# sun-huangqingbo/multiplexed-image-annotator

Hardware: AMD Instinct MI355X
Metric: cells/sec annotated (whole node) (higher is better)
Workload: dtype f16

## Files before the change

multiplexed-image-annotator_amd/csrc/cell_attention.hip:

```cpp

#include "gemm_epi.h"
#include "ribca_common.h"
#include "ribca_kernels.h"

namespace ribca {

namespace {

typedef __attribute__((__vector_size__(4 * sizeof(_Float16)))) _Float16 f16x4c;
typedef __attribute__((__vector_size__(4 * sizeof(short)))) short s16x4c;
__device__ __forceinline__ f16x4c lds_read_tr16c(const char* p) {
  return __builtin_bit_cast(f16x4c, __builtin_amdgcn_ds_read_tr16_b64_v4i16((s16x4c __attribute__((address_space(3)))*)(p)));
}

constexpr int kTP = 112, kVRows = 128;

template <int D, int HD> struct CellGeom {
  static constexpr int Dp = (D + 31) / 32 * 32;
  static constexpr int NK = Dp / 32;
  static constexpr int GD = HD == 32 ? 64 : 48;
  static constexpr int NTP = GD / 16;
  static constexpr int WROWS = 3 * GD;
  static constexpr int WSTAGE = WROWS * ROWB;
  static constexpr int GROUPS = D / GD;
  static constexpr int HPG = GD / HD;
  static constexpr int KIMG = kTP * ROWB;
  static constexpr int VROWB = 4 * GD;
  static constexpr int VIMG = kVRows * VROWB + 64;
  static constexpr int CB = 2 * 3 * D * 4;
  static constexpr int RING = 3;
  static constexpr int OFF_K = RING * WSTAGE;
  static constexpr int OFF_V = OFF_K + HPG * KIMG;
  static constexpr int OFF_CB = OFF_V + (VIMG + 15) / 16 * 16;
  static constexpr int LDS = OFF_CB + CB;
  static_assert(D % GD == 0 && GD % HD == 0 && HD % 4 == 0 && HD <= 32 && HPG % 2 == 0 && WROWS % 8 == 0, "head geometry");
};

}

template <int D, int HD>
__global__ __launch_bounds__(512) void cell_qkv_attention_kernel(const uint16_t* __restrict__ z, int ldz, const uint16_t* __restrict__ W, int ldw,
                                                                 const float* __restrict__ bias2, const float* __restrict__ csum,
                                                                 const float2* __restrict__ rowstat, uint16_t* __restrict__ out, int ldo, int T,
                                                                 float scale) {
  using G = CellGeom<D, HD>;
  constexpr int NK = G::NK, GROUPS = G::GROUPS, HPG = G::HPG, kRing = G::RING, kGroupDims = G::GD, NTP = G::NTP, kWStage = G::WSTAGE;
  constexpr int NTILES = 3 * NTP;
  constexpr int TOTAL = GROUPS * NK;
  constexpr int GPL = G::WROWS / 8;
  extern __shared__ __attribute__((aligned(16))) char smem[];
  const int tid = threadIdx.x, lane = tid & 63;
  const int wave = __builtin_amdgcn_readfirstlane(tid >> 6);
  const int cell = blockIdx.x;
  const int r16 = lane & 15, g = lane >> 4;

  for (int i = tid; i < 3 * D / 4; i += 512) {
    reinterpret_cast<float4*>(smem + G::OFF_CB)[i] = reinterpret_cast<const float4*>(csum)[i];
    reinterpret_cast<float4*>(smem + G::OFF_CB + 3 * D * 4)[i] = reinterpret_cast<const float4*>(bias2)[i];
  }
  for (int o = kTP * G::VROWB + tid * 16; o < G::VIMG; o += 512 * 16) *reinterpret_cast<uint4*>(smem + G::OFF_V + o) = uint4{0u, 0u, 0u, 0u};
  __syncthreads();

  if (wave == 7) {
    auto issue = [&](int step) {
      const int hg = step / NK, s = step - hg * NK;
      char* st = smem + (step % kRing) * kWStage;
#pragma unroll
      for (int i = 0; i < GPL; ++i) {
        const int row = i * 8 + (lane >> 3);
        const int which = row / kGroupDims, c = row - which * kGroupDims;
        const int n = which * D + hg * kGroupDims + c;
        const int ch = (lane & 7) ^ swz_f(row);
        const uint16_t* src = W + (size_t)n * ldw + s * (2 * BK) + ch * 8;
        __builtin_amdgcn_global_load_lds((const __attribute__((address_space(1))) void*)src, (__attribute__((address_space(3))) void*)(st + i * 1024), 16,
                                         0, 0);
      }
    };
    issue(0);
    issue(1);
    for (int step = 0; step < TOTAL; ++step) {
      if (step + 1 < TOTAL) wait_vmcnt<GPL>();
      else wait_vmcnt<0>();
      __builtin_amdgcn_s_barrier();
      asm volatile("" ::: "memory");
      if (step + 2 < TOTAL) issue(step + 2);
      if ((step + 1) % NK == 0) __builtin_amdgcn_s_barrier();
    }
    return;
  }

  const int tok = wave * 16 + r16;
  const int trow = tok < T ? tok : T - 1;
  const uint16_t* zr = z + ((size_t)cell * T + trow) * ldz;
  f16x8 ahi[NK], alo[NK];
#pragma unroll
  for (int s = 0; s < NK; ++s) {
    const uint4* p = reinterpret_cast<const uint4*>(zr + (4 * s + g) * 16);
    ahi[s] = __builtin_bit_cast(f16x8, p[0]);
    alo[s] = __builtin_bit_cast(f16x8, p[1]);
  }
  const float2 rs = rowstat[(size_t)cell * T + trow];
  const float rstd = rs.x, nm = -rs.y * rs.x;
  const char* cb = smem + G::OFF_CB;
  uint16_t* orow = out + ((size_t)cell * T + tok) * ldo;
  int w_rd[NTILES];
#pragma unroll
  for (int j = 0; j < NTILES; ++j) w_rd[j] = lds_off(16 * j + r16, 2 * g);
  const int k_wr = lds_off(tok, 2 * g);
  constexpr int KST = 4, NT = 7;

  int step = 0;
  for (int hg = 0; hg < GROUPS; ++hg) {
    f32x4 acc[NTILES];
#pragma unroll
    for (int j = 0; j < NTILES; ++j) acc[j] = f32x4{0.f, 0.f, 0.f, 0.f};
#pragma unroll
    for (int s = 0; s < NK; ++s, ++step) {
      asm volatile("s_waitcnt lgkmcnt(0)" ::: "memory");
      __builtin_amdgcn_s_barrier();
      asm volatile("" ::: "memory");
      const char* st = smem + (step % kRing) * kWStage;
#pragma unroll
      for (int jb = 0; jb < NTILES / 3; ++jb) {
        f16x8 whi[3], wlo[3];
#pragma unroll
        for (int j = 0; j < 3; ++j) {
          whi[j] = __builtin_bit_cast(f16x8, *reinterpret_cast<const uint4*>(st + w_rd[3 * jb + j]));
          wlo[j] = __builtin_bit_cast(f16x8, *reinterpret_cast<const uint4*>(st + (w_rd[3 * jb + j] ^ 16)));
        }
#pragma unroll
        for (int j = 0; j < 3; ++j) acc[3 * jb + j] = mfma_f16(wlo[j], ahi[s], acc[3 * jb + j]);
#pragma unroll
        for (int j = 0; j < 3; ++j) acc[3 * jb + j] = mfma_f16(whi[j], alo[s], acc[3 * jb + j]);
#pragma unroll
        for (int j = 0; j < 3; ++j) acc[3 * jb + j] = mfma_f16(whi[j], ahi[s], acc[3 * jb + j]);
      }
    }
#pragma unroll
    for (int j = 0; j < NTILES; ++j) {
      const int n = (j / NTP) * D + hg * kGroupDims + 16 * (j % NTP) + 4 * g;
      const float4 c4 = *reinterpret_cast<const float4*>(cb + n * 4), b4 = *reinterpret_cast<const float4*>(cb + 3 * D * 4 + n * 4);
      const f32x2v r2 = {rstd, rstd}, n2 = {nm, nm};
      const f32x2v lo2 = fma2(r2, f32x2v{acc[j][0], acc[j][1]}, fma2(n2, f32x2v{c4.x, c4.y}, f32x2v{b4.x, b4.y}));
      const f32x2v hi2 = fma2(r2, f32x2v{acc[j][2], acc[j][3]}, fma2(n2, f32x2v{c4.z, c4.w}, f32x2v{b4.z, b4.w}));
      acc[j] = f32x4{lo2.x, lo2.y, hi2.x, hi2.y};
    }
    f16x8 qhi[HPG], qlo[HPG];
#pragma unroll
    for (int h = 0; h < HPG; ++h) {
      constexpr int dummy = 0; (void)dummy;
      const int d_lo = h * HD, d_hi = d_lo + HD;
      const int tA = d_lo / 16, tB = (d_hi - 1) / 16;
      const bool inA = 16 * tA + 4 * g >= d_lo && 16 * tA + 4 * g < d_hi;
      const bool inB = tB != tA && 16 * tB + 4 * g >= d_lo && 16 * tB + 4 * g < d_hi;
      float qa[4], qb[4], ka[4], kb[4];
#pragma unroll
      for (int r = 0; r < 4; ++r) {
        qa[r] = inA ? acc[tA][r] * scale : 0.f;
        qb[r] = inB ? acc[tB][r] * scale : 0.f;
        ka[r] = inA ? acc[NTP + tA][r] : 0.f;
        kb[r] = inB ? acc[NTP + tB][r] : 0.f;
      }
      uint2 h0, l0, h1, l1;
      split4(qa, h0, l0);
      split4(qb, h1, l1);
      qhi[h] = __builtin_bit_cast(f16x8, uint4{h0.x, h0.y, h1.x, h1.y});
      qlo[h] = __builtin_bit_cast(f16x8, uint4{l0.x, l0.y, l1.x, l1.y});
      split4(ka, h0, l0);
      split4(kb, h1, l1);
      char* kimg = smem + G::OFF_K + h * G::KIMG;
      *reinterpret_cast<uint4*>(kimg + k_wr) = uint4{h0.x, h0.y, h1.x, h1.y};
      *reinterpret_cast<uint4*>(kimg + (k_wr ^ 16)) = uint4{l0.x, l0.y, l1.x, l1.y};
    }
    {
      uint16_t* vrow = reinterpret_cast<uint16_t*>(smem + G::OFF_V + tok * G::VROWB);
#pragma unroll
      for (int j = 0; j < NTP; ++j) {
        const float v4[4] = {acc[2 * NTP + j][0], acc[2 * NTP + j][1], acc[2 * NTP + j][2], acc[2 * NTP + j][3]};
        const int jj = kGroupDims == 64 ? (j ^ (tok & 3)) : j;
        ps_store4_pair<16>(vrow, 16 * jj + 4 * g, v4);
      }
    }
    asm volatile("s_waitcnt lgkmcnt(0)" ::: "memory");
    __builtin_amdgcn_s_barrier();
    asm volatile("" ::: "memory");

    constexpr int DT = (HD + 15) / 16;
    const char* vimg = smem + G::OFF_V;
#pragma unroll
    for (int hp = 0; hp < HPG; hp += 2) {
      f32x4 s[2][2 * KST];
#pragma unroll
      for (int kt = 0; kt < NT; ++kt) {
        const int ko = lds_off(16 * kt + r16, 2 * g);
#pragma unroll
        for (int e = 0; e < 2; ++e) {
          const char* kimg = smem + G::OFF_K + (hp + e) * G::KIMG;
          const f16x8 kh = __builtin_bit_cast(f16x8, *reinterpret_cast<const uint4*>(kimg + ko));
          const f16x8 kl = __builtin_bit_cast(f16x8, *reinterpret_cast<const uint4*>(kimg + (ko ^ 16)));
          s[e][kt] = f32x4{0.f, 0.f, 0.f, 0.f};
          s[e][kt] = mfma_f16(kl, qhi[hp + e], s[e][kt]);
          s[e][kt] = mfma_f16(kh, qlo[hp + e], s[e][kt]);
          s[e][kt] = mfma_f16(kh, qhi[hp + e], s[e][kt]);
        }
      }
      f16x8 phi[2][KST], plo[2][KST];
#pragma unroll
      for (int e = 0; e < 2; ++e) {
#pragma unroll
        for (int r = 0; r < 4; ++r)
          if (16 * (NT - 1) + 4 * g + r >= T) s[e][NT - 1][r] = -INFINITY;
        float mx = -INFINITY;
#pragma unroll
        for (int kt = 0; kt < NT; ++kt)
#pragma unroll
          for (int r = 0; r < 4; ++r) mx = fmaxf(mx, s[e][kt][r]);
        mx = fmaxf(mx, __shfl_xor(mx, 16, 64));
        mx = fmaxf(mx, __shfl_xor(mx, 32, 64));
        const f32x2v l2 = {1.44269504089f, 1.44269504089f}, moff = {-mx * 1.44269504089f, -mx * 1.44269504089f};
        f32x2v sum2 = {0.f, 0.f};
#pragma unroll
        for (int kt = 0; kt < NT; ++kt) {
          const f32x2v a0 = fma2(f32x2v{s[e][kt][0], s[e][kt][1]}, l2, moff);
          const f32x2v a1 = fma2(f32x2v{s[e][kt][2], s[e][kt][3]}, l2, moff);
          const f32x2v e0 = {__builtin_amdgcn_exp2f(a0.x), __builtin_amdgcn_exp2f(a0.y)}, e1 = {__builtin_amdgcn_exp2f(a1.x), __builtin_amdgcn_exp2f(a1.y)};
          s[e][kt] = f32x4{e0.x, e0.y, e1.x, e1.y};
          sum2 += e0;
          sum2 += e1;
        }
        float sum = sum2.x + sum2.y;
        sum += __shfl_xor(sum, 16, 64);
        sum += __shfl_xor(sum, 32, 64);
        const float inv = 1.0f / sum;
        const f32x2v inv2 = {inv, inv};
        s[e][NT] = f32x4{0.f, 0.f, 0.f, 0.f};
#pragma unroll
        for (int t = 0; t < KST; ++t) {
          const f32x2v pa0 = f32x2v{s[e][2 * t][0], s[e][2 * t][1]} * inv2, pa1 = f32x2v{s[e][2 * t][2], s[e][2 * t][3]} * inv2;
          const f32x2v pb0 = f32x2v{s[e][2 * t + 1][0], s[e][2 * t + 1][1]} * inv2, pb1 = f32x2v{s[e][2 * t + 1][2], s[e][2 * t + 1][3]} * inv2;
          const float pa[4] = {pa0.x, pa0.y, pa1.x, pa1.y}, pb[4] = {pb0.x, pb0.y, pb1.x, pb1.y};
          uint2 ha, la, hb, lb;
          split4_unit(pa, ha, la);
          split4_unit(pb, hb, lb);
          phi[e][t] = __builtin_bit_cast(f16x8, uint4{ha.x, ha.y, hb.x, hb.y});
          plo[e][t] = __builtin_bit_cast(f16x8, uint4{la.x, la.y, lb.x, lb.y});
        }
      }
#pragma unroll
      for (int dt = 0; dt < DT; ++dt) {
        f32x4 o[2] = {f32x4{0.f, 0.f, 0.f, 0.f}, f32x4{0.f, 0.f, 0.f, 0.f}};
#pragma unroll
        for (int t = 0; t < KST; ++t) {
#pragma unroll
          for (int e = 0; e < 2; ++e) {
            const int dcol0 = (hp + e) * HD + 16 * dt + 4 * (r16 & 3);
            const int dcol = kGroupDims == 64 ? ((((dcol0 >> 4) ^ (r16 >> 2)) << 4) | (dcol0 & 15)) : dcol0;
            const int voff = (dcol >> 3) * 32 + (dcol & 7) * 2;
            const char* va = vimg + (32 * t + 4 * g + (r16 >> 2)) * G::VROWB + voff;
            const f16x4c h0 = lds_read_tr16c(va), l0 = lds_read_tr16c(va + 16);
            const f16x4c h1 = lds_read_tr16c(va + 16 * G::VROWB), l1 = lds_read_tr16c(va + 16 * G::VROWB + 16);
            const f16x8 vhi = __builtin_shufflevector(h0, h1, 0, 1, 2, 3, 4, 5, 6, 7);
            const f16x8 vlo = __builtin_shufflevector(l0, l1, 0, 1, 2, 3, 4, 5, 6, 7);
            o[e] = mfma_f16(vlo, phi[e][t], o[e]);
            o[e] = mfma_f16(vhi, plo[e][t], o[e]);
            o[e] = mfma_f16(vhi, phi[e][t], o[e]);
          }
        }
        const int d = 16 * dt + 4 * g;
        if (tok < T && d < HD) {
#pragma unroll
          for (int e = 0; e < 2; ++e) {
            const float v4[4] = {o[e][0], o[e][1], o[e][2], o[e][3]};
            ps_store4(orow, (hg * HPG + hp + e) * HD + d, v4);
          }
        }
      }
    }
  }
}

bool cell_attention_supported(int D, int H, int T) { return H == kHeads && T == kTokens && (D == 144 || D == 288 || D == 384); }

void launch_cell_qkv_attention(const uint16_t* z, int ldz, const uint16_t* W, int ldw, const float* bias2, const float* csum, const float2* rowstat,
                               uint16_t* out, int ldo, int cells, int D, float scale, hipStream_t s) {
  if (cells <= 0) return;
  auto go = [&](auto kern, int lds) {
    static unsigned long long attr_done[3] = {0ull, 0ull, 0ull};
    const int slot = D == 288 ? 1 : D == 384 ? 2 : 0;
    if (!ensure_dynamic_lds(reinterpret_cast<const void*>(kern), lds, attr_done[slot])) return;
    hipLaunchKernelGGL(kern, dim3(cells), dim3(512), lds, s, z, ldz, W, ldw, bias2, csum, rowstat, out, ldo, (int)kTokens, scale);
  };
  if (D == 288) go(cell_qkv_attention_kernel<288, 24>, CellGeom<288, 24>::LDS);
  else if (D == 384) go(cell_qkv_attention_kernel<384, 32>, CellGeom<384, 32>::LDS);
  else go(cell_qkv_attention_kernel<144, 12>, CellGeom<144, 12>::LDS);
}

}
```

Measured before the change: 17400.

## Make cell attention kernel persistent and deepen weight ring for HD=24

Launches one workgroup per CU, and each workgroup loops over cells with a grid stride. The loader wave streams weights continuously across cell boundaries, so the ring no longer refills from empty for every cell. For HD=24 the ring grows to 5 stages, with counted vmcnt waits that keep more loads in flight, and LDS address arithmetic is simplified. The costs are more LDS use, which static asserts check against 160 KB, and fewer resident blocks, which may hurt load balance at the tail.

```diff
diff --git a/multiplexed-image-annotator_amd/csrc/cell_attention.hip b/multiplexed-image-annotator_amd/csrc/cell_attention.hip
--- a/multiplexed-image-annotator_amd/csrc/cell_attention.hip
+++ b/multiplexed-image-annotator_amd/csrc/cell_attention.hip
@@ -1,3 +1,5 @@
+
+#include <type_traits>
 
 #include "gemm_epi.h"
 #include "ribca_common.h"
@@ -28,12 +30,14 @@
   static constexpr int VROWB = 4 * GD;
   static constexpr int VIMG = kVRows * VROWB + 64;
   static constexpr int CB = 2 * 3 * D * 4;
-  static constexpr int RING = 3;
+  static constexpr int RING = HD == 24 ? 5 : 3;
   static constexpr int OFF_K = RING * WSTAGE;
   static constexpr int OFF_V = OFF_K + HPG * KIMG;
   static constexpr int OFF_CB = OFF_V + (VIMG + 15) / 16 * 16;
   static constexpr int LDS = OFF_CB + CB;
   static_assert(D % GD == 0 && GD % HD == 0 && HD % 4 == 0 && HD <= 32 && HPG % 2 == 0 && WROWS % 8 == 0, "head geometry");
+  static_assert(LDS <= 160 * 1024, "one workgroup per CU: the ring, the K / V images and the fold vectors share 160 KB of LDS");
+  static_assert(RING >= 3 && (RING - 2) * (WROWS / 8) <= 63 && NK >= RING - 2, "the loader's counted wait: RING - 2 younger stages in a 6-bit vmcnt");
 };
 
 }
@@ -42,16 +46,16 @@
 __global__ __launch_bounds__(512) void cell_qkv_attention_kernel(const uint16_t* __restrict__ z, int ldz, const uint16_t* __restrict__ W, int ldw,
                                                                  const float* __restrict__ bias2, const float* __restrict__ csum,
                                                                  const float2* __restrict__ rowstat, uint16_t* __restrict__ out, int ldo, int T,
-                                                                 float scale) {
+                                                                 int cells, float scale) {
   using G = CellGeom<D, HD>;
   constexpr int NK = G::NK, GROUPS = G::GROUPS, HPG = G::HPG, kRing = G::RING, kGroupDims = G::GD, NTP = G::NTP, kWStage = G::WSTAGE;
   constexpr int NTILES = 3 * NTP;
-  constexpr int TOTAL = GROUPS * NK;
   constexpr int GPL = G::WROWS / 8;
+  constexpr int kTopUp = kRing - 3;
   extern __shared__ __attribute__((aligned(16))) char smem[];
   const int tid = threadIdx.x, lane = tid & 63;
   const int wave = __builtin_amdgcn_readfirstlane(tid >> 6);
-  const int cell = blockIdx.x;
+  const int cell0 = blockIdx.x, cstride = gridDim.x;
   const int r16 = lane & 15, g = lane >> 4;
 
   for (int i = tid; i < 3 * D / 4; i += 512) {
@@ -62,37 +66,62 @@
   __syncthreads();
 
   if (wave == 7) {
-    auto issue = [&](int step) {
-      const int hg = step / NK, s = step - hg * NK;
-      char* st = smem + (step % kRing) * kWStage;
+    const int total = ((cells - 1 - cell0) / cstride + 1) * (GROUPS * NK);
+    int issued = 0, i_slot = 0, i_hg = 0, i_s = 0;
+    auto issue = [&]() {
+      if (issued == total) return;
+      char* st = smem + i_slot * kWStage;
 #pragma unroll
       for (int i = 0; i < GPL; ++i) {
         const int row = i * 8 + (lane >> 3);
         const int which = row / kGroupDims, c = row - which * kGroupDims;
-        const int n = which * D + hg * kGroupDims + c;
+        const int n = which * D + i_hg * kGroupDims + c;
         const int ch = (lane & 7) ^ swz_f(row);
-        const uint16_t* src = W + (size_t)n * ldw + s * (2 * BK) + ch * 8;
+        const uint16_t* src = W + (size_t)n * ldw + i_s * (2 * BK) + ch * 8;
         __builtin_amdgcn_global_load_lds((const __attribute__((address_space(1))) void*)src, (__attribute__((address_space(3))) void*)(st + i * 1024), 16,
                                          0, 0);
       }
+      ++issued;
+      i_slot = i_slot + 1 == kRing ? 0 : i_slot + 1;
+      if (++i_s == NK) {
+        i_s = 0;
+        i_hg = i_hg + 1 == GROUPS ? 0 : i_hg + 1;
+      }
     };
-    issue(0);
-    issue(1);
-    for (int step = 0; step < TOTAL; ++step) {
-      if (step + 1 < TOTAL) wait_vmcnt<GPL>();
-      else wait_vmcnt<0>();
+#pragma unroll
+    for (int e = 0; e < kRing - 1; ++e) issue();
+    auto step_barrier = [&](auto younger, bool request) {
+      if (issued == total) wait_vmcnt<0>();
+      else wait_vmcnt<decltype(younger)::value * GPL>();
       __builtin_amdgcn_s_barrier();
       asm volatile("" ::: "memory");
-      if (step + 2 < TOTAL) issue(step + 2);
-      if ((step + 1) % NK == 0) __builtin_amdgcn_s_barrier();
+      if (request) issue();
+    };
+    static_assert(kTopUp >= 0 && kTopUp <= 2, "the lead-draining steps are written out below");
+    for (int left = total; left > 0; left -= NK) {
+      if constexpr (kTopUp >= 1) step_barrier(std::integral_constant<int, kRing - 2>{}, false);
+      if constexpr (kTopUp >= 2) step_barrier(std::integral_constant<int, kRing - 3>{}, false);
+#pragma unroll
+      for (int i = kTopUp; i < NK; ++i) step_barrier(std::integral_constant<int, 1>{}, true);
+      __builtin_amdgcn_s_barrier();
+      asm volatile("" ::: "memory");
+#pragma unroll
+      for (int e = 0; e < kTopUp; ++e) issue();
     }
     return;
   }
 
   const int tok = wave * 16 + r16;
   const int trow = tok < T ? tok : T - 1;
+  f16x8 ahi[NK], alo[NK];
+  const char* cb = smem + G::OFF_CB;
+  const int w_rd0 = lds_off(r16, 2 * g), w_rd1 = w_rd0 ^ 16;
+  const int k_wr = lds_off(tok, 2 * g);
+  constexpr int KST = 4, NT = 7;
+
+  int slot = 0;
+  for (int cell = cell0; cell < cells; cell += cstride) {
   const uint16_t* zr = z + ((size_t)cell * T + trow) * ldz;
-  f16x8 ahi[NK], alo[NK];
 #pragma unroll
   for (int s = 0; s < NK; ++s) {
     const uint4* p = reinterpret_cast<const uint4*>(zr + (4 * s + g) * 16);
@@ -100,33 +129,29 @@
     alo[s] = __builtin_bit_cast(f16x8, p[1]);
   }
   const float2 rs = rowstat[(size_t)cell * T + trow];
-  const float rstd = rs.x, nm = -rs.y * rs.x;
-  const char* cb = smem + G::OFF_CB;
+  float rstd = rs.x, nm = -rs.y * rs.x;
+#pragma unroll
+  for (int s = 0; s < NK; ++s) asm volatile("" : "+v"(ahi[s]), "+v"(alo[s]));
+  asm volatile("" : "+v"(rstd), "+v"(nm));
   uint16_t* orow = out + ((size_t)cell * T + tok) * ldo;
-  int w_rd[NTILES];
-#pragma unroll
-  for (int j = 0; j < NTILES; ++j) w_rd[j] = lds_off(16 * j + r16, 2 * g);
-  const int k_wr = lds_off(tok, 2 * g);
-  constexpr int KST = 4, NT = 7;
-
-  int step = 0;
   for (int hg = 0; hg < GROUPS; ++hg) {
     f32x4 acc[NTILES];
 #pragma unroll
     for (int j = 0; j < NTILES; ++j) acc[j] = f32x4{0.f, 0.f, 0.f, 0.f};
 #pragma unroll
-    for (int s = 0; s < NK; ++s, ++step) {
+    for (int s = 0; s < NK; ++s) {
       asm volatile("s_waitcnt lgkmcnt(0)" ::: "memory");
       __builtin_amdgcn_s_barrier();
       asm volatile("" ::: "memory");
-      const char* st = smem + (step % kRing) * kWStage;
+      const char* st = smem + slot * kWStage;
+      slot = slot + 1 == kRing ? 0 : slot + 1;
 #pragma unroll
       for (int jb = 0; jb < NTILES / 3; ++jb) {
         f16x8 whi[3], wlo[3];
 #pragma unroll
         for (int j = 0; j < 3; ++j) {
-          whi[j] = __builtin_bit_cast(f16x8, *reinterpret_cast<const uint4*>(st + w_rd[3 * jb + j]));
-          wlo[j] = __builtin_bit_cast(f16x8, *reinterpret_cast<const uint4*>(st + (w_rd[3 * jb + j] ^ 16)));
+          whi[j] = __builtin_bit_cast(f16x8, *reinterpret_cast<const uint4*>(st + w_rd0 + (3 * jb + j) * 16 * ROWB));
+          wlo[j] = __builtin_bit_cast(f16x8, *reinterpret_cast<const uint4*>(st + w_rd1 + (3 * jb + j) * 16 * ROWB));
         }
 #pragma unroll
         for (int j = 0; j < 3; ++j) acc[3 * jb + j] = mfma_f16(wlo[j], ahi[s], acc[3 * jb + j]);
@@ -192,12 +217,11 @@
       f32x4 s[2][2 * KST];
 #pragma unroll
       for (int kt = 0; kt < NT; ++kt) {
-        const int ko = lds_off(16 * kt + r16, 2 * g);
 #pragma unroll
         for (int e = 0; e < 2; ++e) {
           const char* kimg = smem + G::OFF_K + (hp + e) * G::KIMG;
-          const f16x8 kh = __builtin_bit_cast(f16x8, *reinterpret_cast<const uint4*>(kimg + ko));
-          const f16x8 kl = __builtin_bit_cast(f16x8, *reinterpret_cast<const uint4*>(kimg + (ko ^ 16)));
+          const f16x8 kh = __builtin_bit_cast(f16x8, *reinterpret_cast<const uint4*>(kimg + w_rd0 + kt * 16 * ROWB));
+          const f16x8 kl = __builtin_bit_cast(f16x8, *reinterpret_cast<const uint4*>(kimg + w_rd1 + kt * 16 * ROWB));
           s[e][kt] = f32x4{0.f, 0.f, 0.f, 0.f};
           s[e][kt] = mfma_f16(kl, qhi[hp + e], s[e][kt]);
           s[e][kt] = mfma_f16(kh, qlo[hp + e], s[e][kt]);
@@ -277,9 +301,25 @@
       }
     }
   }
+  }
 }
 
 bool cell_attention_supported(int D, int H, int T) { return H == kHeads && T == kTokens && (D == 144 || D == 288 || D == 384); }
+
+static int device_cu_count() {
+  static int cached[64] = {};
+  int dev = 0;
+  if (hipGetDevice(&dev) != hipSuccess) dev = 0;
+  if (dev >= 0 && dev < 64 && cached[dev] > 0) return cached[dev];
+  int n = 0;
+  const hipError_t e = hipDeviceGetAttribute(&n, hipDeviceAttributeMultiprocessorCount, dev);
+  if (e != hipSuccess || n <= 0) {
+    launch_error("hipDeviceGetAttribute(MultiprocessorCount) failed on device %d: %s", dev, hipGetErrorString(e));
+    return 0;
+  }
+  if (dev >= 0 && dev < 64) cached[dev] = n;
+  return n;
+}
 
 void launch_cell_qkv_attention(const uint16_t* z, int ldz, const uint16_t* W, int ldw, const float* bias2, const float* csum, const float2* rowstat,
                                uint16_t* out, int ldo, int cells, int D, float scale, hipStream_t s) {
@@ -288,7 +328,9 @@
     static unsigned long long attr_done[3] = {0ull, 0ull, 0ull};
     const int slot = D == 288 ? 1 : D == 384 ? 2 : 0;
     if (!ensure_dynamic_lds(reinterpret_cast<const void*>(kern), lds, attr_done[slot])) return;
-    hipLaunchKernelGGL(kern, dim3(cells), dim3(512), lds, s, z, ldz, W, ldw, bias2, csum, rowstat, out, ldo, (int)kTokens, scale);
+    const int cus = device_cu_count();
+    if (cus <= 0) return;
+    hipLaunchKernelGGL(kern, dim3(cells < cus ? cells : cus), dim3(512), lds, s, z, ldz, W, ldw, bias2, csum, rowstat, out, ldo, (int)kTokens, cells, scale);
   };
   if (D == 288) go(cell_qkv_attention_kernel<288, 24>, CellGeom<288, 24>::LDS);
   else if (D == 384) go(cell_qkv_attention_kernel<384, 32>, CellGeom<384, 32>::LDS);
```

After: 17440 (median of 2 runs). No clear change (+0.2%).
